# GreatAttractor/gpuart

Measured on AMD Instinct MI355X. Metric: Mrays/s (BVH queries EXECUTED by the timed fast mode: camera + bounce + Sun-shadow rays, device-counted; the reference-defined count is in mrays_reference_defined_per_s), path tracing, 1 path/pixel/pass, higher is better.
Workload: dtype f32

## Files before the change

gpuart_amd/csrc/hip/gpuart_hip.hip:

```cpp
#include <dlfcn.h>
#include <hip/hip_runtime.h>

#include <algorithm>
#include <atomic>
#include <chrono>
#include <thread>
#include <utility>
#include <cmath>
#include <cstdio>
#include <cstdlib>
#include <cstring>
#include <new>
#include <string>
#include <vector>

#include "device_shade.h"
#include "gpuart_hip.h"
#include "gpuart_hip_test.h"

#include "kernels_pipeline.h"
#include "kernel_run.h"
#include "kernels_query.h"
#ifdef GPUART_HIP_TEST_HOOKS
#include "kernels_test.h"
// ... 19 lines not shown
    do {                                                                                           \
        hipError_t e_ = (expr);                                                                    \
        if (e_ != hipSuccess)                                                                      \
            return fail(GPUART_HIP_ERR_DEVICE, std::string(#expr) + ": " + hipGetErrorString(e_)); \
    } while (0)

void plane_coef(float x0, float y0, float x1, float y1, float x2, float y2, float a0, float a1, float a2, float c[3]) {
    float x0c = x0 - 0.5f, y0c = y0 - 0.5f;
    float dx01 = x0 - x1, dy01 = y0 - y1, dx20 = x2 - x0, dy20 = y2 - y0;
    float e = dx01 * dy20, f = dy01 * dx20;
    float ooa = 1.0f / (e - f);
    float dy20o = dy20 * ooa, dy01o = dy01 * ooa, dx20o = dx20 * ooa, dx01o = dx01 * ooa;
    float da01 = a0 - a1, da20 = a2 - a0;
    float dadx = da01 * dy20o - da20 * dy01o;
    float dady = da20 * dx01o - da01 * dx20o;
    c[0] = a0 - (dadx * x0c + dady * y0c);
    c[1] = dadx;
    c[2] = dady;
}

struct TimedLaunch {
    hipEvent_t start, stop;
    int cls;
};

}

struct PassLane {
    hipStream_t main = nullptr;
    PathBuffers pb{};
    void *pathmem = nullptr;
    float4 *passcolor = nullptr;
    uint4 *spill_main = nullptr;
    uint32_t counter_segments = 0;
    uint32_t *run_cursor = nullptr;
    hipEvent_t ev_done = nullptr;
    hipEvent_t ev_free = nullptr;
    bool used = false;
};

struct gpuart_hip_ctx {
    int device = 0;
    hipStream_t stream = nullptr;
    Frame frame{};
    bool have_camera = false, have_scene = false;
    bool empty_share = false;
    float4 *d_recs = nullptr, *d_prims = nullptr;
    uint32_t *d_cursor = nullptr;
    uint32_t *d_query_cursor = nullptr;
    uint2 *d_tile_xy = nullptr;
    uint4 *d_spill = nullptr;
    uint32_t *d_tile_order[2] = {nullptr, nullptr};
    uint32_t *d_tile_cost = nullptr;
    hipEvent_t ev_order = nullptr;
    int order_cur = -1, order_next = 0;
    bool order_sorting = false;
    bool order_stale = true;
    bool order_auto = true;
    bool order_from_hook = false;
    std::vector<PassLane> lanes;
    uint32_t next_lane = 0;
    uint32_t spill_levels = 0;
    uint32_t num_cus = 256;
    uint32_t grid_waves = 4096;
    uint32_t direct_waves = 4096;
    uint32_t shade_waves = 4096;
    uint32_t run_waves = 5120;
    TraceTuning tune{128, 16, 16, 3};
    bool lean_kernels = true;
    std::vector<float4> pend_seeds;
    gpuart_params pend_params{};
    int pend_npaths = 0;
    uint64_t n_nodes = 0, n_prims = 0, scene_bytes = 0;
    uint32_t ref_order = 0;
    uint32_t nearest_min_prims = 0xffffffffu;
    uint32_t type_mask = 0;
    float root_min[3] = {0, 0, 0}, root_max[3] = {0, 0, 0};
    uint32_t root_ref = 0;
    bool chunk_from_env = false;
    float box_slack = __builtin_inff();
    uint32_t quick_boxes = 1;
    uint32_t packet = 2;
    uint32_t packet_max_prims = 1u << 19;
    uint32_t exact_boxes = 0;
    uint32_t max_depth = 0;
    float4 *d_direct = nullptr, *d_accum = nullptr;
    unsigned long long *d_counters = nullptr;
    RunPlanner plan;
    std::vector<TimedLaunch> pending, free_events;
    double timed_ms[2] = {0, 0};
    uint64_t timed_launches[2] = {0, 0};
    int timing_level = 1;
    float *d_scratch = nullptr;
    size_t scratch_bytes = 0;
    ncclComm_t comm = nullptr;
    int comm_rank = 0, comm_nranks = 0;
    bool comm_owned = false;
    float4 *d_send = nullptr, *d_stage = nullptr;
    size_t send_pixels = 0, stage_pixels = 0;
    void *d_hello = nullptr;
    void *h_frame = nullptr;
    size_t h_frame_bytes = 0;
    void *h_hello = nullptr;
    uint64_t comm_group = 0;
    uint32_t gather_timeout_ms = 60000;
    bool abandoned = false;
#ifdef GPUART_HIP_TEST_HOOKS
    std::vector<const void *> launched;
#endif
};

namespace {

#ifdef GPUART_HIP_TEST_HOOKS
void ledger_note(gpuart_hip_ctx *c, const void *kernel) {
    if (std::find(c->launched.begin(), c->launched.end(), kernel) == c->launched.end()) c->launched.push_back(kernel);
}
#define GD_LEDGER(c, ...) ledger_note((c), reinterpret_cast<const void *>(&__VA_ARGS__))
#else
#define GD_LEDGER(c, ...) ((void)0)
#endif

enum { KC_DIRECT = 0, KC_RUN = 1, KC_TRACE = 2, KC_QUERY = 3 };
enum { KC_COUNT = 0x100, KC_REFWORK = 0x200 };

int kernel_choice(uint32_t type_mask, bool exact_boxes, bool ref_order, bool lean_kernels, int mode, int entry) {
    const int run = entry != KC_RUN ? 0 : mode == 1 ? KC_COUNT | KC_REFWORK : mode == 4 ? KC_COUNT : 0;
    if (exact_boxes) return run | GD_ALL_TYPES | GD_EXACT_BOXES;
    if (run & KC_REFWORK) return run | GD_ALL_TYPES;
    const bool flat = lean_kernels && (type_mask & ~(uint32_t)GD_FLAT_TYPES) == 0;
    const bool round = lean_kernels && (type_mask & ~(uint32_t)GD_ROUND_TYPES) == 0 && !run;
    const int types = flat ? GD_FLAT_TYPES : round ? GD_ROUND_TYPES : GD_ALL_TYPES;
    return run | types | (ref_order && (entry == KC_RUN || entry == KC_TRACE) ? GD_REF_ORDER : 0);
}
int kernel_choice(const gpuart_hip_ctx *c, int entry) {
    return kernel_choice(c->type_mask, c->exact_boxes != 0, c->ref_order != 0, c->lean_kernels, c->plan.mode, entry);
}

template <int... T> using TypeList = std::integer_sequence<int, T...>;
using LeafTypes = TypeList<GD_FLAT_TYPES, GD_ROUND_TYPES, GD_ALL_TYPES, GD_ALL_TYPES | GD_EXACT_BOXES>;
using TraceTypes = TypeList<GD_FLAT_TYPES, GD_ROUND_TYPES, GD_ALL_TYPES, GD_ALL_TYPES | GD_EXACT_BOXES, GD_FLAT_TYPES | GD_REF_ORDER,
                            GD_ROUND_TYPES | GD_REF_ORDER, GD_ALL_TYPES | GD_REF_ORDER>;
using RunTypes = TypeList<GD_FLAT_TYPES, GD_ROUND_TYPES, GD_ALL_TYPES, GD_ALL_TYPES | GD_EXACT_BOXES, GD_FLAT_TYPES | GD_REF_ORDER,
                          GD_ROUND_TYPES | GD_REF_ORDER, GD_ALL_TYPES | GD_REF_ORDER, KC_COUNT | GD_FLAT_TYPES, KC_COUNT | GD_ALL_TYPES,
                          KC_COUNT | GD_ALL_TYPES | GD_EXACT_BOXES, KC_COUNT | GD_FLAT_TYPES | GD_REF_ORDER, KC_COUNT | GD_ALL_TYPES | GD_REF_ORDER,
                          KC_COUNT | KC_REFWORK | GD_ALL_TYPES, KC_COUNT | KC_REFWORK | GD_ALL_TYPES | GD_EXACT_BOXES>;

template <int... T, class Launch>
int with_types(int choice, TypeList<T...>, const char *kernel, Launch launch) {
    if (((choice == T && (launch(std::integral_constant<int, T>()), true)) || ...)) return 0;
    return fail(GPUART_HIP_ERR_DEVICE, std::string("internal: no ") + kernel + " for choice " + std::to_string(choice));
}

int drain(gpuart_hip_ctx *c) {
    for (auto &l : c->lanes) {
        if (l.main) HIP_TRY(hipStreamSynchronize(l.main));
    }
    HIP_TRY(hipStreamSynchronize(c->stream));
    c->next_lane = 0;
    return 0;
}


int wait_stream(gpuart_hip_ctx *c, uint32_t timeout_ms, const char *what) {
    const auto t0 = std::chrono::steady_clock::now();
    for (;;) {
// ... 169 lines not shown
    HIP_TRY(hipMemsetAsync(dst, 0, bytes, c->stream));
    if (!v.empty()) HIP_TRY(hipMemcpyAsync(dst, v.data(), v.size() * sizeof(T), hipMemcpyHostToDevice, c->stream));
    HIP_TRY(hipStreamSynchronize(c->stream));
    return 0;
}

int ensure_scratch(gpuart_hip_ctx *c, size_t bytes) {
    if (c->scratch_bytes >= bytes) return 0;
    if (c->d_scratch) (void)hipFree(c->d_scratch);
    c->d_scratch = nullptr;
    c->scratch_bytes = 0;
    HIP_TRY(hipMalloc(&c->d_scratch, bytes));
    c->scratch_bytes = bytes;
    return 0;
}

template <class Launch>
int run_hook(gpuart_hip_ctx *c, int n, const float *const *ins, int nin, float *const *outs, int nout, Launch launch) {
    if (!c || n < 0) return fail(GPUART_HIP_ERR_ARG, "bad argument");
    if (n == 0) return 0;
    HIP_TRY(hipSetDevice(c->device));
    size_t one = (size_t)n * 16;
    int r = ensure_scratch(c, one * (nin + nout));
    if (r) return r;
    float4 *base = (float4 *)c->d_scratch;
    std::vector<float4 *> di, dout;
    for (int k = 0; k < nin; k++) {
        di.push_back(base + (size_t)k * n);
        HIP_TRY(hipMemcpyAsync(di[k], ins[k], one, hipMemcpyHostToDevice, c->stream));
    }
    for (int k = 0; k < nout; k++) dout.push_back(base + (size_t)(nin + k) * n);
    launch(di, dout);
    HIP_TRY(hipGetLastError());
    for (int k = 0; k < nout; k++) HIP_TRY(hipMemcpyAsync(outs[k], dout[k], one, hipMemcpyDeviceToHost, c->stream));
    HIP_TRY(hipStreamSynchronize(c->stream));
    return 0;
}

}

extern "C" {

const char *gpuart_hip_last_error(void) { return g_last_error.c_str(); }

int gpuart_hip_destroy(gpuart_hip_ctx *c);
static int comm_drop(gpuart_hip_ctx *c);

int gpuart_hip_create(int device, gpuart_hip_ctx **out) {
    if (!out) return fail(GPUART_HIP_ERR_ARG, "out == NULL");
    *out = nullptr;
    int count = 0;
    if (hipGetDeviceCount(&count) != hipSuccess || count <= 0) return fail(GPUART_HIP_ERR_NO_DEVICE, "no HIP device");
    if (device < 0 || device >= count) return fail(GPUART_HIP_ERR_ARG, "device index out of range");
    HIP_TRY(hipSetDevice(device));
    hipDeviceProp_t prop;
    HIP_TRY(hipGetDeviceProperties(&prop, device));
    if (strncmp(prop.gcnArchName, "gfx950", 6) != 0)
        return fail(GPUART_HIP_ERR_NO_DEVICE, std::string("device is ") + prop.gcnArchName + ", this library is built for gfx950 only");
    gpuart_hip_ctx *c = new (std::nothrow) gpuart_hip_ctx();
    if (!c) return fail(GPUART_HIP_ERR_DEVICE, "out of host memory");
    c->device = device;
    auto env_u32 = [](const char *name, uint32_t dflt, uint32_t lo, uint32_t hi) {
        const char *v = getenv(name);
        if (!v) return dflt;
        long x = strtol(v, nullptr, 10);
        return (uint32_t)std::min<long>(hi, std::max<long>(lo, x));
    };
    c->num_cus = prop.multiProcessorCount > 0 ? (uint32_t)prop.multiProcessorCount : 256u;
    c->grid_waves = c->num_cus * env_u32("GPUART_HIP_WAVES_PER_CU", 8, 1, 32);
    c->direct_waves = c->num_cus * env_u32("GPUART_HIP_DIRECT_WAVES_PER_CU", 16, 1, 32);
    c->shade_waves = c->num_cus * env_u32("GPUART_HIP_SHADE_WAVES_PER_CU", 24, 1, 64);
    c->run_waves = c->num_cus * env_u32("GPUART_HIP_RUN_WAVES_PER_CU", 4 * GD_RUN_WAVES, 1, 32);
    c->tune.chunk = env_u32("GPUART_HIP_CHUNK", 128, 16, 4096);
    c->chunk_from_env = getenv("GPUART_HIP_CHUNK") != nullptr;
    c->tune.refill_lanes = env_u32("GPUART_HIP_REFILL_LANES", 16, 1, 64);
    c->tune.leaf_lanes = env_u32("GPUART_HIP_LEAF_LANES", 16, 1, 64);
    c->tune.leaf_share = env_u32("GPUART_HIP_LEAF_SHARE", 3, 1, 64);
    c->tune.xcd_queues = env_u32("GPUART_HIP_XCD_QUEUES", 0, 0, 1);
    c->order_auto = env_u32("GPUART_HIP_TILE_ORDER", 1, 0, 1) != 0;
    c->nearest_min_prims = getenv("GPUART_HIP_NEAREST_MIN_PRIMS") ? env_u32("GPUART_HIP_NEAREST_MIN_PRIMS", 1024, 0, 0x7fffffff) : 0xffffffffu;
    c->quick_boxes = env_u32("GPUART_HIP_QUICK_BOXES", 1, 0, 1);
    c->packet = env_u32("GPUART_HIP_PACKET", 2, 0, 2);
    c->packet_max_prims = env_u32("GPUART_HIP_PACKET_MAX_PRIMS", 1u << 19, 0, 0xffffffffu);
    if (hipStreamCreateWithFlags(&c->stream, hipStreamNonBlocking) != hipSuccess) { delete c; return fail(GPUART_HIP_ERR_DEVICE, "hipStreamCreate failed"); }
    c->lanes.resize(env_u32("GPUART_HIP_PASSES_IN_FLIGHT", 8, 1, 32));
    c->plan.lanes_total = (uint32_t)c->lanes.size();
    c->plan.batch_limit = env_u32("GPUART_HIP_MAX_BATCH", MAX_BATCH, 1, MAX_BATCH);
    c->plan.batch_paths = (size_t)env_u32("GPUART_HIP_BATCH_MPATHS", 16, 1, 256) << 20;
    c->plan.plan_run_factor = env_u32("GPUART_HIP_PLAN_RUN_PERCENT", 0, 0, 1000) / 100.0;
    c->lean_kernels = env_u32("GPUART_HIP_LEAN_KERNELS", 1, 0, 1) != 0;
    c->plan.min_run_paths = (size_t)env_u32("GPUART_HIP_MIN_RUN_KPATHS", 2048, 64, 65536) << 10;
    c->plan.lane_budget = (size_t)env_u32("GPUART_HIP_LANE_BUDGET_MB", 32768, 64, 262144) << 20;
    c->plan.small_paths = (size_t)env_u32("GPUART_HIP_SMALL_KPATHS", 8500, 0, 1 << 20) << 10;
    c->gather_timeout_ms = env_u32("GPUART_HIP_GATHER_TIMEOUT_MS", 60000, 0, 3600000);
    for (auto &l : c->lanes) {
        if (hipStreamCreateWithFlags(&l.main, hipStreamNonBlocking) != hipSuccess ||
            hipEventCreateWithFlags(&l.ev_done, hipEventDisableTiming) != hipSuccess ||
            hipEventCreateWithFlags(&l.ev_free, hipEventDisableTiming) != hipSuccess) {
            gpuart_hip_destroy(c);
            return fail(GPUART_HIP_ERR_DEVICE, "stream / event creation failed");
        }
    }
    if (hipMalloc(&c->d_counters, 16 * sizeof(unsigned long long)) != hipSuccess ||
        hipMemsetAsync(c->d_counters, 0, 16 * sizeof(unsigned long long), c->stream) != hipSuccess) {
        (void)hipStreamDestroy(c->stream); delete c; return fail(GPUART_HIP_ERR_DEVICE, "counter allocation failed");
    }
    *out = c;
    return 0;
}

int gpuart_hip_destroy(gpuart_hip_ctx *c) {
    if (!c) return 0;
    (void)hipSetDevice(c->device);
    c->pend_seeds.clear();
    if (c->abandoned || bounded_ns::stuck().load()) {
        if (wait_stream(c, std::min<uint32_t>(c->gather_timeout_ms ? c->gather_timeout_ms : 2000u, 2000u), "gpuart_hip_destroy"))
            return fail(GPUART_HIP_ERR_TIMEOUT, "gpuart_hip_destroy: the context's stream never drained (a gather was abandoned); the context is leaked, not freed");
        c->abandoned = false;
    }
    (void)drain(c);
    for (auto &t : c->pending) { (void)hipEventDestroy(t.start); (void)hipEventDestroy(t.stop); }
    for (auto &t : c->free_events) { (void)hipEventDestroy(t.start); (void)hipEventDestroy(t.stop); }
    for (auto &l : c->lanes) {
        if (l.ev_done) (void)hipEventDestroy(l.ev_done);
        if (l.ev_free) (void)hipEventDestroy(l.ev_free);
        void *lp[] = {l.pathmem, l.spill_main, l.pb.counters, l.run_cursor};
        for (void *p : lp) if (p) (void)hipFree(p);
        if (l.main) (void)hipStreamDestroy(l.main);
    }
    const bool comm_stuck = bounded_ns::stuck().load();
    if (c->comm && !comm_stuck) (void)comm_drop(c);
    void *ptrs[] = {c->d_recs, c->d_prims, c->d_spill, c->d_direct, c->d_accum, c->d_counters, c->d_scratch, c->d_cursor,
                    c->d_query_cursor, c->d_tile_order[0], c->d_tile_order[1], c->d_tile_cost, c->d_tile_xy};
    for (void *p : ptrs) if (p) (void)hipFree(p);
    void *comm_ptrs[] = {c->d_send, c->d_stage, c->d_hello};
    for (void *p : comm_ptrs) if (p && !comm_stuck) (void)hipFree(p);
    if (c->ev_order) (void)hipEventDestroy(c->ev_order);
    if (c->h_hello && !comm_stuck) (void)hipHostFree(c->h_hello);
    if (c->h_frame && !comm_stuck) (void)hipHostFree(c->h_frame);
    if (c->stream) (void)hipStreamDestroy(c->stream);
    delete c;
    return 0;
}

int gpuart_hip_resize(gpuart_hip_ctx *c, uint32_t width, uint32_t height) {
    if (!c || width == 0 || height == 0 || width > 65536 || height > 65536) return fail(GPUART_HIP_ERR_ARG, "bad frame size");
    HIP_TRY(hipSetDevice(c->device));
    c->frame.W = width; c->frame.H = height;
    c->frame.x0 = 0; c->frame.y0 = 0; c->frame.tw = width; c->frame.th = height;
    c->frame.band_rows = height; c->frame.band_stride = height;
    update_uv(c);
    return realloc_tile(c);
}

int gpuart_hip_set_tile(gpuart_hip_ctx *c, uint32_t x0, uint32_t y0, uint32_t tw, uint32_t th) {
    if (!c || !c->frame.W) return fail(GPUART_HIP_ERR_ARG, "set_tile before resize");
    if (tw == 0 || th == 0 || (uint64_t)x0 + tw > c->frame.W || (uint64_t)y0 + th > c->frame.H)
        return fail(GPUART_HIP_ERR_ARG, "tile outside the frame");
    HIP_TRY(hipSetDevice(c->device));
    c->frame.x0 = x0; c->frame.y0 = y0; c->frame.tw = tw; c->frame.th = th;
    c->frame.band_rows = th; c->frame.band_stride = th;
    return realloc_tile(c);
}

int gpuart_hip_set_tile_interleaved(gpuart_hip_ctx *c, uint32_t x0, uint32_t y0, uint32_t tw, uint32_t th_local,
                                    uint32_t band_rows, uint32_t band_stride) {
// ... 165 lines not shown
    k_tile_order<<<1, TO_THREADS, 0, l.main>>>(c->d_tile_cost, c->d_tile_order[c->order_next], (uint32_t)tiles);
    HIP_TRY(hipGetLastError());
    HIP_TRY(hipEventRecord(c->ev_order, l.main));
    c->order_sorting = true;
    c->order_stale = false;
    return 0;
}

int finish_run(gpuart_hip_ctx *c, PassLane &l, bool gathers) {
    int r;
    HIP_TRY(hipEventRecord(l.ev_done, l.main));
    HIP_TRY(hipStreamWaitEvent(c->stream, l.ev_done, 0));
    GD_LEDGER(c, k_accumulate);
    k_accumulate<<<dim3((unsigned)((c->plan.tile_pixels + 255) / 256)), 256, 0, c->stream>>>(c->d_accum, l.passcolor, c->plan.tile_pixels, l.pb.batch);
    HIP_TRY(hipGetLastError());
    HIP_TRY(hipEventRecord(l.ev_free, c->stream));
    if (gathers && (r = sort_tile_order(c, l))) return r;
    l.used = true;
    return 0;
}

int launch_run_persistent(gpuart_hip_ctx *c, PassLane &l, size_t first, size_t count) {
    int r;
    const gpuart_params *p = &c->pend_params;
    const int npaths = c->pend_npaths;
    Scene sc = scene_of(c);
    SeedBatch seeds{};
    for (size_t k = 0; k < count; k++) seeds.seed[k] = c->pend_seeds[first + k];
    if (!l.run_cursor) HIP_TRY(hipMalloc(&l.run_cursor, 64));
    const PathBuffers &b = l.pb;
    if ((uint64_t)b.n_slots * b.batch > (uint64_t)RUN_SLOT + 1)
        return fail(GPUART_HIP_ERR_ARG, "modes 1, 4 and 5 run through k_run, whose list entries address 2^28 path slots per run; this tile has " +
                    std::to_string((uint64_t)b.n_slots * b.batch) + " (use mode 0 or 3, or a smaller tile)");
    const uint32_t chunks = b.n_slots * b.batch / BLOCK;
    const dim3 grid(std::min<uint32_t>(c->run_waves, std::max<uint32_t>(1, chunks)));
    TimedLaunch t;
    Frame fr;
    bool gathers;
    if ((r = run_frame(c, fr, gathers, count == 1))) return r;
    if (l.used) HIP_TRY(hipStreamWaitEvent(l.main, l.ev_free, 0));
    if ((r = begin_timed(c, t, 0, l.main))) return r;
    for (int j = 0; j < npaths; j++) {
        TimedLaunch tt;
        HIP_TRY(hipMemsetAsync(l.run_cursor, 0, sizeof(uint32_t), l.main));
        if (c->timing_level >= 2 && (r = begin_timed(c, tt, 1, l.main))) return r;
        if ((r = with_types(kernel_choice(c, KC_RUN), RunTypes(), "k_run", [&](auto K) {
                constexpr bool C = (K() & KC_COUNT) != 0, R = (K() & KC_REFWORK) != 0;
                constexpr int T = K() & (KC_COUNT - 1);
                GD_LEDGER(c, k_run<C, R, T>);
                k_run<C, R, T><<<grid, BLOCK, 0, l.main>>>(sc, fr, *p, seeds, b, j, npaths, l.passcolor, l.spill_main, c->d_counters, c->tune, l.run_cursor);
            })))
            return r;
        if (c->timing_level >= 2 && (r = end_timed(c, tt, l.main))) return r;
    }
    if ((r = end_timed(c, t, l.main))) return r;
    return finish_run(c, l, gathers);
}

int launch_run(gpuart_hip_ctx *c, size_t first, size_t count) {
    int r;
    const gpuart_params *p = &c->pend_params;
    const int npaths = c->pend_npaths;
    Scene sc = scene_of(c);
    TimedLaunch t;
    if (const char *bad = c->plan.check(count)) return fail(GPUART_HIP_ERR_DEVICE, std::string("internal: ") + bad);
    PassLane &l = c->lanes[c->next_lane];
    c->next_lane = (c->next_lane + 1) % c->plan.lanes_in_use;
    l.pb.batch = (uint32_t)count;
    if (c->plan.uses_run_kernel(count)) return launch_run_persistent(c, l, first, count);
    const uint32_t nseg = segment_bound(c, p);
    SeedBatch seeds{};
    for (size_t k = 0; k < count; k++) seeds.seed[k] = c->pend_seeds[first + k];
    if ((r = ensure_segment_counters(c, l, nseg))) return r;
    const PathBuffers &b = l.pb;
    const bool detail = c->timing_level >= 2;
    const dim3 pgrid(c->grid_waves);
    const dim3 sgrid(std::min<uint32_t>(c->shade_waves, b.n_slots * b.batch / BLOCK));
    int j_cur = 0;
    Frame fr;
    bool gathers;
    if ((r = run_frame(c, fr, gathers, false))) return r;
    if (l.used) HIP_TRY(hipStreamWaitEvent(l.main, l.ev_free, 0));
    if ((r = begin_timed(c, t, 0, l.main))) return r;
    auto trace = [&](int seg_c, int seg_s) -> int {
        TimedLaunch tt;
        int rr;
        if (detail && (rr = begin_timed(c, tt, 1, l.main))) return rr;
        TraceTuning tune = c->tune;
        const uint32_t packet = c->n_prims <= c->packet_max_prims ? c->packet : 0u;
        tune.packet = (packet >= 1 && seg_c == 0) ? 1u : (packet >= 2 && seg_s == 0) ? 2u : 0u;
        if ((rr = with_types(kernel_choice(c, KC_TRACE), TraceTypes(), "k_trace", [&](auto T) {
                GD_LEDGER(c, k_trace<false, T()>);
                k_trace<false, T()><<<pgrid, BLOCK, 0, l.main>>>(sc, fr, *p, b, seg_c, seg_s, 1, j_cur, npaths, l.passcolor, l.spill_main, c->d_counters, tune);
            })))
            return rr;
        if (detail && (rr = end_timed(c, tt, l.main))) return rr;
        return 0;
    };
    for (int j = 0; j < npaths; j++) {
        j_cur = j;
        HIP_TRY(hipMemsetAsync(b.counters, 0, 4 * ((size_t)nseg + 1) * sizeof(uint32_t), l.main));
        if (c->tune.xcd_queues) HIP_TRY(hipMemsetAsync(b.xcd_cursors, 0, 16 * ((size_t)nseg + 1) * sizeof(uint32_t), l.main));
        GD_LEDGER(c, k_gen);
        k_gen<<<sgrid, BLOCK, 0, l.main>>>(fr, *p, seeds, j, npaths, b, l.passcolor);
        if (nseg && (r = trace(0, -1))) return r;
        for (uint32_t seg = 0; seg < nseg; seg++) {
            GD_LEDGER(c, k_shade<false>);
            k_shade<false><<<sgrid, BLOCK, 0, l.main>>>(sc, fr, *p, seeds, b, (int)seg, (int)nseg, j, npaths, l.passcolor, c->d_counters);
            const int next_c = seg + 1 < nseg ? (int)seg + 1 : -1, sh = p->sunEnabled == 1 ? (int)seg : -1;
            if ((next_c >= 0 || sh >= 0) && (r = trace(next_c, sh))) return r;
        }
        HIP_TRY(hipGetLastError());
    }
    if ((r = end_timed(c, t, l.main))) return r;
    return finish_run(c, l, gathers);
}
}
}

int gpuart_hip_flush(gpuart_hip_ctx *c) {
    if (!c) return fail(GPUART_HIP_ERR_ARG, "ctx == NULL");
    const size_t pending = c->pend_seeds.size();
    if (!pending) return 0;
    HIP_TRY(hipSetDevice(c->device));
    c->plan.pending = pending;
    int r = 0;
    size_t first = 0;
    for (size_t count : c->plan.on_flush()) {
        if ((r = launch_run(c, first, count))) break;
        first += count;
    }
    c->pend_seeds.clear();
    return r;
}


int gpuart_hip_pt_pass(gpuart_hip_ctx *c, const gpuart_params *p, const float randSeed[4], int npaths) {
    int r = check_ready(c, p);
    if (r) return r > 0 ? 0 : r;
    if (!randSeed || npaths < 0) return fail(GPUART_HIP_ERR_ARG, "bad argument");
    if (p->maxSegments > GPUART_HIP_MAX_SEGMENTS) return fail(GPUART_HIP_ERR_ARG, "maxSegments exceeds GPUART_HIP_MAX_SEGMENTS");
    if (npaths == 0) return 0;
    HIP_TRY(hipSetDevice(c->device));
    const float4 seed = make_float4(randSeed[0], randSeed[1], randSeed[2], randSeed[3]);
    if (c->plan.mode == 2) {
        if ((r = gpuart_hip_flush(c))) return r;
        Scene sc = scene_of(c);
        TimedLaunch t;
        if ((r = begin_timed(c, t, 0))) return r;
        dim3 grid(std::min<uint32_t>(c->grid_waves, c->plan.n_slots / BLOCK));
        GD_LEDGER(c, k_pt_mega<false>);
        k_pt_mega<false><<<grid, BLOCK, 0, c->stream>>>(sc, c->frame, *p, seed, npaths, c->plan.n_slots, c->d_accum, c->d_spill, c->d_counters);
        HIP_TRY(hipGetLastError());
        return end_timed(c, t);
    }
    if (!c->pend_seeds.empty() && (memcmp(&c->pend_params, p, sizeof *p) != 0 || c->pend_npaths != npaths))
        if ((r = gpuart_hip_flush(c))) return r;
    c->pend_params = *p;
    c->pend_npaths = npaths;
    c->pend_seeds.push_back(seed);
    c->plan.pending = c->pend_seeds.size() - 1;
    if (const size_t count = c->plan.on_pass()) {
        r = launch_run(c, 0, count);
        c->pend_seeds.clear();
        return r;
    }
    return 0;
}

int gpuart_hip_export(gpuart_hip_ctx *c, int which, void *rgba_device, float divide_by) {
    if (!c || !rgba_device || (which != 0 && which != 1) || !c->plan.tile_pixels) return fail(GPUART_HIP_ERR_ARG, "bad argument");
    HIP_TRY(hipSetDevice(c->device));
    { int fr = gpuart_hip_flush(c); if (fr) return fr; }
    const float4 *src = which == 0 ? c->d_direct : c->d_accum;
    if (!(divide_by > 0)) divide_by = 1.0f;
    size_t n = c->plan.tile_pixels;
    GD_LEDGER(c, k_scale_copy);
    k_scale_copy<<<dim3((unsigned)((n + 255) / 256)), 256, 0, c->stream>>>(src, (float4 *)rgba_device, n, divide_by);
    HIP_TRY(hipGetLastError());
    return 0;
}

int gpuart_hip_read(gpuart_hip_ctx *c, int which, float *rgba_host, float divide_by) {
    if (!c || !rgba_host || (which != 0 && which != 1) || !c->plan.tile_pixels) return fail(GPUART_HIP_ERR_ARG, "bad argument");
    HIP_TRY(hipSetDevice(c->device));
    { int fr = gpuart_hip_flush(c); if (fr) return fr; }
    size_t bytes = c->plan.tile_pixels * sizeof(float4);
    const float4 *src = which == 0 ? c->d_direct : c->d_accum;
// ... 978 lines not shown
```

gpuart_amd/csrc/hip/kernels_pipeline.h:

```cpp
#pragma once
#include <hip/hip_runtime.h>

#include <type_traits>

#include "device_shade.h"
#include "gpuart_hip.h"

using namespace gd;

#define BLOCK 64
#define SHADE_ROUNDS 8

struct TraceTuning {
    uint32_t chunk;
    uint32_t refill_lanes;
    uint32_t leaf_lanes;
    uint32_t leaf_share;
    uint32_t xcd_queues;
    uint32_t packet;
};

namespace {

#ifdef GD_STEP_STATS
// ... 109 lines not shown
GD_FN TravStack make_stack(uint2 *ring_a, float *ring_b, uint4 *spill, uint32_t total_lanes, uint32_t wave, uint32_t column) {
    TravStack st;
    st.ring_a = ring_a + column;
    st.ring_b = ring_b + column;
    st.ring_stride = BLOCK;
    st.spill = spill + (size_t)wave * BLOCK + column;
    st.spill_stride = total_lanes;
    st.reset();
    return st;
}
GD_FN TravStack make_stack(uint2 *ring_a, float *ring_b, uint4 *spill, uint32_t total_lanes, uint32_t wave) {
    return make_stack(ring_a, ring_b, spill, total_lanes, wave, (uint32_t)lane_id());
}
GD_FN TravStack make_stack(uint2 *ring_a, float *ring_b, uint4 *spill, uint32_t total_lanes) {
    return make_stack(ring_a, ring_b, spill, total_lanes, blockIdx.x);
}

GD_FN void thin_regroup(uint32_t to, unsigned long long flying, uint32_t *xfer, uint2 *ring_a, float *ring_b, uint4 *spill,
                        uint32_t &tag0, uint32_t &tag1, F3 &ro, F3 &rd, F3 &rdiv, Trav &t, TravStack &st, int *src_lane = nullptr) {
    if ((flying >> lane_id()) & 1ull) xfer[__popcll(flying & ((1ull << lane_id()) - 1))] = (uint32_t)lane_id();
    __builtin_amdgcn_fence(__ATOMIC_ACQ_REL, "workgroup");
    const uint32_t q = (uint32_t)lane_id() / to;
    const bool holds = q < (uint32_t)__popcll(flying);
    const int src = holds ? (int)xfer[q] : lane_id();
    if (src_lane) *src_lane = src;
    tag0 = __shfl(tag0, src, 64); tag1 = __shfl(tag1, src, 64);
    ro = f3(__shfl(ro.x, src, 64), __shfl(ro.y, src, 64), __shfl(ro.z, src, 64));
    rd = f3(__shfl(rd.x, src, 64), __shfl(rd.y, src, 64), __shfl(rd.z, src, 64));
    rdiv = f3(__shfl(rdiv.x, src, 64), __shfl(rdiv.y, src, 64), __shfl(rdiv.z, src, 64));
    t.closest = __shfl(t.closest, src, 64); t.hit_prim = __shfl(t.hit_prim, src, 64); t.node = __shfl(t.node, src, 64);
    t.entry = __shfl(t.entry, src, 64); t.state = __shfl(t.state, src, 64); t.second = __shfl(t.second, src, 64);
    uint32_t sp = __shfl(st.sp, src, 64), base = __shfl(st.base, src, 64);
    if (!holds) { t.state = TRAV_DONE; sp = 0; base = 0; }
    const bool mover = holds && ((uint32_t)lane_id() % to) == 0 && src != lane_id();
    for (uint32_t k = 0; k < GD_RING; k++) {
        const uint2 a = ring_a[k * BLOCK + (uint32_t)src];
        const float bb = ring_b[k * BLOCK + (uint32_t)src];
        if (mover) { ring_a[k * BLOCK + lane_id()] = a; ring_b[k * BLOCK + lane_id()] = bb; }
    }
    for (uint32_t k = 0; __ballot(mover && k < base) != 0; k++) {
        const bool mv = mover && k < base;
        uint4 v = make_uint4(0, 0, 0, 0);
        const size_t row = (size_t)k * gridDim.x * BLOCK + (size_t)blockIdx.x * BLOCK;
        if (mv) v = spill[row + (uint32_t)src];
        if (mv) spill[row + lane_id()] = v;
    }
    __builtin_amdgcn_fence(__ATOMIC_ACQ_REL, "workgroup");
    st = make_stack(ring_a, ring_b, spill, gridDim.x * BLOCK, blockIdx.x, (uint32_t)lane_id() / to * to);
    st.sp = sp; st.base = base;
}

GD_FN void queue_push(uint32_t *queue, uint32_t *counter, bool pred, uint32_t value) {
    unsigned long long m = __ballot(pred);
    if (!m) return;
    uint32_t base = 0;
    int leader = __ffsll((long long)m) - 1;
    if (lane_id() == leader) base = atomicAdd(counter, (uint32_t)__popcll(m));
    base = __shfl(base, leader, 64);
    if (pred) queue[base + (uint32_t)__popcll(m & ((1ull << lane_id()) - 1))] = value;
}

GD_FN void path_commit(const Frame &f, const PathBuffers &b, float4 *passcolor, uint32_t slot, int j, int npaths, F3 value) {
    F3 c = (j == 0) ? f3(0.0f + value.x, 0.0f + value.y, 0.0f + value.z) : xyz(b.color[slot]) + value;
    if (j == npaths - 1) {
        uint32_t lx, ly;
        slot_pixel(f, slot_pixel_slot(b, slot), lx, ly);
        passcolor[(size_t)slot_pass(b, slot) * b.tile_pixels + (size_t)ly * f.tw + lx] = make_float4(c.x, c.y, c.z, 0);
    } else
        b.color[slot] = make_float4(c.x, c.y, c.z, 0);
}

__global__ void k_accumulate(float4 *__restrict__ accum, const float4 *__restrict__ passcolor, size_t n, uint32_t batch) {
    size_t i = (size_t)blockIdx.x * blockDim.x + threadIdx.x;
    if (i < n) {
        float4 a = accum[i];
        for (uint32_t k = 0; k < batch; k++) {
            float4 c = passcolor[(size_t)k * n + i];
            a = make_float4(a.x + c.x, a.y + c.y, a.z + c.z, a.w);
        }
        accum[i] = a;
    }
}

__global__ void __launch_bounds__(BLOCK) k_gen(Frame f, gpuart_params P, SeedBatch seeds, int j, int npaths, PathBuffers b,
                                               float4 *accum) {
    const bool no_segments = !(P.maxSegments > 0 && 1.0f > P.minWeight);
    const uint32_t total = b.n_slots * b.batch;
    for (uint32_t slot = blockIdx.x * BLOCK + threadIdx.x; slot < total; slot += gridDim.x * BLOCK) {
        uint32_t lx, ly;
        bool valid = slot_pixel(f, slot_pixel_slot(b, slot), lx, ly);
        const float4 seed = seeds.seed[slot_pass(b, slot)];
        uint32_t q = SLOT_INVALID;
        if (valid) {
            F3 rs0, rd0, rs, rd;
            camera_ray(f, f.x0 + lx, frame_y(f, ly), rs0, rd0);
            if (no_segments) {
                path_commit(f, b, accum, slot, j, npaths, path_finish(P, rd0, 0, false, false, f3(0, 0, 0)));
            } else {
                path_begin(P, seed, j, rs0, rd0, rs, rd);
                b.ray_o[slot] = make_float4(rs.x, rs.y, rs.z, 0);
                b.ray_d[slot] = make_float4(rd.x, rd.y, rd.z, 0);
                q = slot;
            }
        }
        b.queue[0][slot] = q;
    }
    if (blockIdx.x == 0 && threadIdx.x == 0) b.counters[0] = no_segments ? 0u : total;
}

#define GD_FLAT_TYPES ((1 << gd::P_DISC) | (1 << gd::P_TRIANGLE))
#define GD_ROUND_TYPES ((1 << gd::P_SPHERE) | (1 << gd::P_DISC))
#define GD_LEAN_TYPES(T) (((T) & ~GD_REF_ORDER) == GD_FLAT_TYPES || ((T) & ~GD_REF_ORDER) == GD_ROUND_TYPES)
#ifndef GD_TRACE_WAVES
#define GD_TRACE_WAVES 5
#endif
#ifndef GD_TRACE_THIN
#define GD_TRACE_THIN 4
#endif
#ifndef GD_TRACE_WAVES_LEAN
#define GD_TRACE_WAVES_LEAN 6
#endif
struct ChunkCursor {
    uint32_t next, end, static_end, n;
    bool exhausted;
    GD_FN ChunkCursor(uint32_t n_, uint32_t chunk)
        : next(min(blockIdx.x * chunk, n_)), end(min((blockIdx.x + 1) * chunk, n_)), static_end(gridDim.x * chunk), n(n_), exhausted(false) {}
    GD_FN uint32_t take(unsigned long long idle, bool lane_idle, uint32_t *cursor, uint32_t chunk, bool &served) {
        served = false;
        if (next == end) {
            if (static_end >= n) { exhausted = true; return SLOT_INVALID; }
            uint32_t base = 0;
            if (lane_id() == 0) base = atomicAdd(cursor, chunk);
            base = wave_value(base) + static_end;
            if (base >= n) { exhausted = true; return SLOT_INVALID; }
            next = base;
            end = min(base + chunk, n);
        }
        const uint32_t want = (uint32_t)__popcll(idle), got = min(want, end - next);
        const uint32_t rank = (uint32_t)__popcll(idle & ((1ull << lane_id()) - 1));
        const uint32_t entry = lane_idle && rank < got ? next + rank : SLOT_INVALID;
        next += got;
        served = got == want;
        return entry;
    }
};

#define GD_THIN_WIDTH(left) ((left) <= BLOCK / 4 && GD_TRACE_THIN >= 4 ? 4u : (left) <= BLOCK / 2 ? 2u : 1u)

template <int TYPES, bool NEAR, class Stop>
GD_FN void wide_rounds(const Scene &sc, const F3 &ro, const F3 &rd, const F3 &rdiv, Trav &t, TravStack &st, const TraceTuning &tune,
                       bool follow, Stop stop) {
    for (;;) {
        if (t.state == TRAV_DESCEND) trav_step_box<false, GD_BOXES_OF(TYPES), NEAR>(sc, Ray{ro, rd}, rdiv, t, st, nullptr, follow);
        unsigned long long at_leaf = __ballot((t.state & 1) != 0);
        unsigned long long descending = __ballot(t.state == TRAV_DESCEND);
        const uint32_t waiting = (uint32_t)__popcll(at_leaf);
        if (at_leaf && (waiting >= tune.leaf_lanes || tune.leaf_share * waiting >= waiting + (uint32_t)__popcll(descending))) {
            if (t.state & 1) {
                trav_step_leaf<false, false, TYPES, NEAR>(sc, Ray{ro, rd}, t, st, nullptr, follow);
                if (stop()) t.state = TRAV_DONE;
            }
            descending = __ballot(t.state == TRAV_DESCEND);
            at_leaf = __ballot((t.state & 1) != 0);
        }
        const unsigned long long busy = descending | at_leaf;
        if (!busy) break;
        if (64u - (uint32_t)__popcll(busy) >= tune.refill_lanes) break;
    }
}

template <int W, int TYPES, bool NEAR, class Stop>
GD_FN void thin_rounds(const Scene &sc, const F3 &ro, const F3 &rd, const F3 &rdiv, Trav &t, TravStack &st, uint32_t sub, bool holds,
                       const TraceTuning &tune, bool follow, Stop stop) {
    constexpr unsigned long long LEAD = W == 4 ? 0x1111111111111111ull : 0x5555555555555555ull;
    for (;;) {
        if (t.state == TRAV_DESCEND) trav_step_box_thin<W, NEAR>(sc, ro, rd, rdiv, t, st, sub, follow);
        const unsigned long long at_leaf = __ballot((t.state & 1) != 0) & LEAD;
        unsigned long long busy = __ballot(t.state != TRAV_DONE) & LEAD;
        const uint32_t waiting = (uint32_t)__popcll(at_leaf);
        if (at_leaf && (W * waiting >= tune.leaf_lanes || tune.leaf_share * waiting >= (uint32_t)__popcll(busy))) {
            if (t.state & 1) {
                trav_step_leaf_thin<W, TYPES, NEAR>(sc, ro, rd, t, st, sub, follow);
                if (stop()) t.state = TRAV_DONE;
            }
            busy = __ballot(t.state != TRAV_DONE) & LEAD;
        }
        if (!busy) break;
        const uint32_t answered = (uint32_t)__popcll(__ballot(holds && t.state == TRAV_DONE) & LEAD);
        if (2 * answered >= (uint32_t)__popcll(busy)) break;
    }
}

template <bool COUNT, int TYPES>
__global__ void __launch_bounds__(BLOCK, GD_LEAN_TYPES(TYPES) ? GD_TRACE_WAVES_LEAN : GD_TRACE_WAVES)
k_trace(Scene sc, Frame f, gpuart_params P, PathBuffers b, int seg_c, int seg_s, int any_shadow, int j, int npaths, float4 *accum,
        uint4 *spill, unsigned long long *gcounters, TraceTuning tune) {
    __shared__ uint2 ring_a[GD_RING * BLOCK];
    __shared__ float ring_b[GD_RING * BLOCK];
    const uint32_t wave_id = blockIdx.x, n_waves = gridDim.x;
    TravStack st = make_stack(ring_a, ring_b, spill, n_waves * BLOCK, wave_id);
    constexpr bool THIN_OK = GD_TRACE_THIN > 1 && !COUNT && GD_BOXES_OF(TYPES) == GD_BOXES_FAST;
    constexpr bool NEAR = GD_NEAREST_OF(TYPES) && !COUNT;
    uint32_t M = 1, sub = 0;
    const uint32_t *queue_c = b.queue[seg_c & 1];
    const uint32_t n_c = seg_c >= 0 ? b.counters[4 * seg_c] : 0u;
    constexpr bool PACKET_OK = !COUNT && (TYPES & GD_REF_ORDER) && GD_BOXES_OF(TYPES) == GD_BOXES_FAST;
    const uint32_t packet = PACKET_OK ? tune.packet : 0u;
    const uint32_t sh_base = packet == 2 ? (n_c + 63u) & ~63u : n_c;
    const uint32_t n = sh_base + (seg_s >= 0 ? b.counters[4 * seg_s + 2] : 0u);
    const uint32_t p_lo = packet == 1 ? 0u : packet == 2 ? sh_base : n;
    uint32_t *cursor = &b.counters[seg_c >= 0 ? 4 * seg_c + 1 : 4 * seg_s + 3];
    const F3 sun = f3(P.sunDirAlt[0], P.sunDirAlt[1], P.sunDirAlt[2]);
    WorkCounters wc = {0, 0, {0, 0, 0, 0}, 0, 0, 0};

    uint32_t static_end = n_waves * tune.chunk;
    uint32_t chunk_next = min(wave_id * tune.chunk, n), chunk_end = min((wave_id + 1) * tune.chunk, n);
    uint32_t q_end = n;
    if (tune.xcd_queues) {
        const uint32_t xcd = wave_id & 7u, wx = wave_id >> 3, nwx = (n_waves + 7u - xcd) >> 3;
        const uint32_t lo = (uint32_t)((unsigned long long)n * xcd / 8u);
        q_end = (uint32_t)((unsigned long long)n * (xcd + 1u) / 8u);
        chunk_next = min(lo + wx * tune.chunk, q_end); chunk_end = min(lo + (wx + 1) * tune.chunk, q_end);
        static_end = lo + nwx * tune.chunk;
        cursor = &b.xcd_cursors[16 * (seg_c >= 0 ? seg_c : seg_s) + (seg_c >= 0 ? 0 : 8) + xcd];
    }
    bool exhausted = false;
    uint32_t slot = SLOT_INVALID;
    bool shadow = false;
    bool refwalk = false;
    F3 ro = f3(0, 0, 0), rd = f3(1, 0, 0);
    F3 rdiv = f3(1, 1, 1);
    Trav t; t.state = TRAV_DONE; t.closest = 0; t.hit_prim = GD_NO_PRIM; t.node = 0; t.entry = 0; t.second = 0;

    auto take_query = [&](uint32_t i) {
        const bool sh = i >= n_c;
        const uint32_t s = !sh ? queue_c[i] : i >= sh_base ? b.shadow_queue[i - sh_base] : SLOT_INVALID;
        if (s != SLOT_INVALID) {
            slot = s;
            shadow = sh;
            refwalk = false;
            ro = xyz(b.ray_o[s]);
            rd = sh ? sun : xyz(b.ray_d[s]);
            rdiv = f3(1 / rd.x, 1 / rd.y, 1 / rd.z);
            trav_init<GD_BOXES_OF(TYPES)>(sc, Ray{ro, rd}, rdiv, t, st, &wc, COUNT, NEAR && !sh);
        }
    };

#ifdef GD_STEP_STATS
    uint32_t ss_box = 0, ss_box_lanes = 0, ss_leaf = 0, ss_leaf_lanes = 0, ss_rounds = 0, ss_held = 0, ss_refills = 0;
    unsigned long long ss_t_refill = 0, ss_t_trav = 0, ss_t_retire = 0, ss_mark = __builtin_amdgcn_s_memtime();
#define GD_SS_PHASE(acc) { const unsigned long long now_ = __builtin_amdgcn_s_memtime(); acc += now_ - ss_mark; ss_mark = now_; }
#else
#define GD_SS_PHASE(acc)
#endif
    for (;;) {
        unsigned long long idle = __ballot(slot == SLOT_INVALID);
#ifdef GD_STEP_STATS
        ss_refills++;
#endif
        bool in_packet = false;
        bool hold = false;
        while (idle && !exhausted) {
            if (chunk_next == chunk_end) {
                if (static_end >= q_end) { exhausted = true; break; }
                uint32_t base = 0;
                if (lane_id() == 0) base = atomicAdd(cursor, tune.chunk);
                base = wave_value(base) + static_end;
                if (base >= q_end) { exhausted = true; break; }
                chunk_next = base;
                chunk_end = min(base + tune.chunk, q_end);
            }
            if (PACKET_OK && chunk_next >= p_lo) {
                if (idle == ~0ull) {
// ... 369 lines not shown
```

Measured before the change: 5961.

## Fuse camera-ray generation with first-hit BVH traversal in k_gen

Ray generation now also traverses the BVH for the camera rays, using packet traversal with chunked work distribution, and writes hits directly. This removes the separate first k_trace launch and the round trip through global ray buffers and queue for camera rays. In exchange, k_gen picks up shared-memory stacks and traversal register pressure, and its grid is sized by chunk count, which may lower occupancy compared with the specialised trace kernel.

Result: faster. 6152, median of 6 (+3.2%).

```diff
diff --git a/gpuart_amd/csrc/hip/gpuart_hip.hip b/gpuart_amd/csrc/hip/gpuart_hip.hip
--- a/gpuart_amd/csrc/hip/gpuart_hip.hip
+++ b/gpuart_amd/csrc/hip/gpuart_hip.hip
@@ -125,6 +125,7 @@
     uint32_t quick_boxes = 1;
     uint32_t packet = 2;
     uint32_t packet_max_prims = 1u << 19;
+    uint32_t gen_walk = 1;
     uint32_t exact_boxes = 0;
     uint32_t max_depth = 0;
     float4 *d_direct = nullptr, *d_accum = nullptr;
@@ -460,6 +461,7 @@
     c->quick_boxes = env_u32("GPUART_HIP_QUICK_BOXES", 1, 0, 1);
     c->packet = env_u32("GPUART_HIP_PACKET", 2, 0, 2);
     c->packet_max_prims = env_u32("GPUART_HIP_PACKET_MAX_PRIMS", 1u << 19, 0, 0xffffffffu);
+    c->gen_walk = env_u32("GPUART_HIP_GEN_WALK", 1, 0, 1);
     if (hipStreamCreateWithFlags(&c->stream, hipStreamNonBlocking) != hipSuccess) { delete c; return fail(GPUART_HIP_ERR_DEVICE, "hipStreamCreate failed"); }
     c->lanes.resize(env_u32("GPUART_HIP_PASSES_IN_FLIGHT", 8, 1, 32));
     c->plan.lanes_total = (uint32_t)c->lanes.size();
@@ -791,14 +793,18 @@
     if ((r = run_frame(c, fr, gathers, false))) return r;
     if (l.used) HIP_TRY(hipStreamWaitEvent(l.main, l.ev_free, 0));
     if ((r = begin_timed(c, t, 0, l.main))) return r;
+    const int trace_choice = kernel_choice(c, KC_TRACE);
+    const uint32_t packet = c->n_prims <= c->packet_max_prims ? c->packet : 0u;
+    const bool gen_walk = c->gen_walk && packet >= 1 && (trace_choice & GD_REF_ORDER) && !(trace_choice & GD_EXACT_BOXES) && nseg > 0 &&
+                          (nseg >= 2 || p->sunEnabled == 1);
+    const dim3 wgrid(std::max<uint32_t>(1u, std::min<uint32_t>(c->grid_waves, (b.n_slots * b.batch + c->tune.chunk - 1) / c->tune.chunk)));
     auto trace = [&](int seg_c, int seg_s) -> int {
         TimedLaunch tt;
         int rr;
         if (detail && (rr = begin_timed(c, tt, 1, l.main))) return rr;
         TraceTuning tune = c->tune;
-        const uint32_t packet = c->n_prims <= c->packet_max_prims ? c->packet : 0u;
         tune.packet = (packet >= 1 && seg_c == 0) ? 1u : (packet >= 2 && seg_s == 0) ? 2u : 0u;
-        if ((rr = with_types(kernel_choice(c, KC_TRACE), TraceTypes(), "k_trace", [&](auto T) {
+        if ((rr = with_types(trace_choice, TraceTypes(), "k_trace", [&](auto T) {
                 GD_LEDGER(c, k_trace<false, T()>);
                 k_trace<false, T()><<<pgrid, BLOCK, 0, l.main>>>(sc, fr, *p, b, seg_c, seg_s, 1, j_cur, npaths, l.passcolor, l.spill_main, c->d_counters, tune);
             })))
@@ -811,8 +817,15 @@
         HIP_TRY(hipMemsetAsync(b.counters, 0, 4 * ((size_t)nseg + 1) * sizeof(uint32_t), l.main));
         if (c->tune.xcd_queues) HIP_TRY(hipMemsetAsync(b.xcd_cursors, 0, 16 * ((size_t)nseg + 1) * sizeof(uint32_t), l.main));
         GD_LEDGER(c, k_gen);
-        k_gen<<<sgrid, BLOCK, 0, l.main>>>(fr, *p, seeds, j, npaths, b, l.passcolor);
-        if (nseg && (r = trace(0, -1))) return r;
+        if (gen_walk) {
+            TimedLaunch tt;
+            if (detail && (r = begin_timed(c, tt, 1, l.main))) return r;
+            k_gen<<<wgrid, BLOCK, 0, l.main>>>(sc, fr, *p, seeds, j, npaths, b, l.passcolor, l.spill_main, c->tune.chunk, trace_choice);
+            if (detail && (r = end_timed(c, tt, l.main))) return r;
+        } else {
+            k_gen<<<sgrid, BLOCK, 0, l.main>>>(sc, fr, *p, seeds, j, npaths, b, l.passcolor, l.spill_main, c->tune.chunk, 0);
+            if (nseg && (r = trace(0, -1))) return r;
+        }
         for (uint32_t seg = 0; seg < nseg; seg++) {
             GD_LEDGER(c, k_shade<false>);
             k_shade<false><<<sgrid, BLOCK, 0, l.main>>>(sc, fr, *p, seeds, b, (int)seg, (int)nseg, j, npaths, l.passcolor, c->d_counters);
diff --git a/gpuart_amd/csrc/hip/kernels_pipeline.h b/gpuart_amd/csrc/hip/kernels_pipeline.h
--- a/gpuart_amd/csrc/hip/kernels_pipeline.h
+++ b/gpuart_amd/csrc/hip/kernels_pipeline.h
@@ -215,32 +215,6 @@
     }
 }
 
-__global__ void __launch_bounds__(BLOCK) k_gen(Frame f, gpuart_params P, SeedBatch seeds, int j, int npaths, PathBuffers b,
-                                               float4 *accum) {
-    const bool no_segments = !(P.maxSegments > 0 && 1.0f > P.minWeight);
-    const uint32_t total = b.n_slots * b.batch;
-    for (uint32_t slot = blockIdx.x * BLOCK + threadIdx.x; slot < total; slot += gridDim.x * BLOCK) {
-        uint32_t lx, ly;
-        bool valid = slot_pixel(f, slot_pixel_slot(b, slot), lx, ly);
-        const float4 seed = seeds.seed[slot_pass(b, slot)];
-        uint32_t q = SLOT_INVALID;
-        if (valid) {
-            F3 rs0, rd0, rs, rd;
-            camera_ray(f, f.x0 + lx, frame_y(f, ly), rs0, rd0);
-            if (no_segments) {
-                path_commit(f, b, accum, slot, j, npaths, path_finish(P, rd0, 0, false, false, f3(0, 0, 0)));
-            } else {
-                path_begin(P, seed, j, rs0, rd0, rs, rd);
-                b.ray_o[slot] = make_float4(rs.x, rs.y, rs.z, 0);
-                b.ray_d[slot] = make_float4(rd.x, rd.y, rd.z, 0);
-                q = slot;
-            }
-        }
-        b.queue[0][slot] = q;
-    }
-    if (blockIdx.x == 0 && threadIdx.x == 0) b.counters[0] = no_segments ? 0u : total;
-}
-
 #define GD_FLAT_TYPES ((1 << gd::P_DISC) | (1 << gd::P_TRIANGLE))
 #define GD_ROUND_TYPES ((1 << gd::P_SPHERE) | (1 << gd::P_DISC))
 #define GD_LEAN_TYPES(T) (((T) & ~GD_REF_ORDER) == GD_FLAT_TYPES || ((T) & ~GD_REF_ORDER) == GD_ROUND_TYPES)
@@ -322,6 +296,60 @@
         const uint32_t answered = (uint32_t)__popcll(__ballot(holds && t.state == TRAV_DONE) & LEAD);
         if (2 * answered >= (uint32_t)__popcll(busy)) break;
     }
+}
+
+__global__ void __launch_bounds__(BLOCK) k_gen(Scene sc, Frame f, gpuart_params P, SeedBatch seeds, int j, int npaths, PathBuffers b,
+                                               float4 *accum, uint4 *spill, uint32_t chunk, int walk) {
+    __shared__ uint2 ring_a[GD_RING * BLOCK];
+    __shared__ float ring_b[GD_RING * BLOCK];
+    const bool no_segments = !(P.maxSegments > 0 && 1.0f > P.minWeight);
+    const uint32_t total = b.n_slots * b.batch;
+    auto first_ray = [&](uint32_t slot, F3 &rs, F3 &rd) {
+        uint32_t lx, ly;
+        bool valid = slot_pixel(f, slot_pixel_slot(b, slot), lx, ly);
+        const float4 seed = seeds.seed[slot_pass(b, slot)];
+        uint32_t q = SLOT_INVALID;
+        if (valid) {
+            F3 rs0, rd0;
+            camera_ray(f, f.x0 + lx, frame_y(f, ly), rs0, rd0);
+            if (no_segments) {
+                path_commit(f, b, accum, slot, j, npaths, path_finish(P, rd0, 0, false, false, f3(0, 0, 0)));
+            } else {
+                path_begin(P, seed, j, rs0, rd0, rs, rd);
+                b.ray_o[slot] = make_float4(rs.x, rs.y, rs.z, 0);
+                b.ray_d[slot] = make_float4(rd.x, rd.y, rd.z, 0);
+                q = slot;
+            }
+        }
+        b.queue[0][slot] = q;
+        return q != SLOT_INVALID;
+    };
+    if (walk == 0) {
+        for (uint32_t slot = blockIdx.x * BLOCK + threadIdx.x; slot < total; slot += gridDim.x * BLOCK) {
+            F3 rs, rd;
+            first_ray(slot, rs, rd);
+        }
+    } else {
+        TravStack st = make_stack(ring_a, ring_b, spill, gridDim.x * BLOCK);
+        ChunkCursor cur(total, chunk);
+        for (;;) {
+            bool served;
+            const uint32_t slot = cur.take(~0ull, true, &b.counters[1], chunk, served);
+            if (cur.exhausted) break;
+            F3 ro = f3(0, 0, 0), rd = f3(1, 0, 0), rdiv = f3(1, 1, 1);
+            Trav t; t.state = TRAV_DONE; t.closest = 0; t.hit_prim = GD_NO_PRIM; t.node = 0; t.entry = 0; t.second = 0;
+            const bool query = slot != SLOT_INVALID && first_ray(slot, ro, rd);
+            if (query) {
+                rdiv = f3(1 / rd.x, 1 / rd.y, 1 / rd.z);
+                trav_init<GD_BOXES_FAST>(sc, Ray{ro, rd}, rdiv, t, st, nullptr, false);
+            }
+            if (walk == (GD_FLAT_TYPES | GD_REF_ORDER)) trav_packet<GD_FLAT_TYPES | GD_REF_ORDER>(sc, ro, rd, rdiv, t, st, false);
+            else if (walk == (GD_ROUND_TYPES | GD_REF_ORDER)) trav_packet<GD_ROUND_TYPES | GD_REF_ORDER>(sc, ro, rd, rdiv, t, st, false);
+            else trav_packet<GD_ALL_TYPES | GD_REF_ORDER>(sc, ro, rd, rdiv, t, st, false);
+            if (query) b.hit[slot] = make_uint2(__float_as_uint(t.closest), t.hit_prim);
+        }
+    }
+    if (blockIdx.x == 0 && threadIdx.x == 0) b.counters[0] = no_segments ? 0u : total;
 }
 
 template <bool COUNT, int TYPES>
```
